# SCUT-BIP-Lab/SplatCo

Hardware: AMD Instinct MI355X
Metric: rasterizer fwd+bwd Msplats/s @1080p; PSNR-match vs ref (higher is better)
Workload: dtype f32; 1 GPU; cfg1: 1M synthetic Gaussians (seed 0), 1 view 1920x1080 per GPU, GaussianRasterizer forward+backward, colors_precomp + scale/rotation path; gaussians=1000000, image=1920x1080, visible=1000000, parallelism=1 view per GPU (mv sharding)

## Files before the change

include/splatco_raster.h:

```cpp
#ifndef SPLATCO_RASTER_H
#define SPLATCO_RASTER_H

#include <stddef.h>
#include <stdint.h>

#ifdef __cplusplus
extern "C" {
#endif

#define SCR_ABI_VERSION 36
#define SCR_TILE 16

typedef struct scr_settings {
    int32_t image_height;
    int32_t image_width;
    float tanfovx;
    float tanfovy;
    const float* bg;
    float scale_modifier;
    const float* viewmatrix;
    const float* projmatrix;
    int32_t sh_degree;
    const float* campos;
    int32_t prefiltered;
// ... 40 lines not shown
                 const void* binning_buf, void* image_buf, const float* dL_dcolor, const float* dL_ddepth,
                 const float* dL_dalpha, void* scratch,
                 float* dL_dmeans3D, float* dL_dmeans2D, float* dL_dcolors, float* dL_dsh,
                 float* dL_dopacity, float* dL_dscales, float* dL_drotations, float* dL_dcov3D,
                 float* dL_dviewmatrix, float* dL_dprojmatrix, float* dL_dcampos, void* stream);

enum {
    SCR_DBG_TILES_TOUCHED = 0,
    SCR_DBG_POINT_OFFSETS = 1,
    SCR_DBG_RANGES = 2,
    SCR_DBG_POINT_LIST = 3,
    SCR_DBG_N_CONTRIB = 4,
    SCR_DBG_FINAL_T = 5,
    SCR_DBG_SPLAT_RECORDS = 6,
    SCR_DBG_QMASK = 7,
    SCR_DBG_GM_INDEX = 8
};
int scr_debug_force_deep_lists(int mode);
int scr_debug_get(int which, int64_t P, int64_t num_rendered, int32_t image_height, int32_t image_width,
                  const void* geom_buf, const void* binning_buf, const void* image_buf, void* out,
                  void* stream);

size_t scr_tpa_scratch_bytes(int32_t R, int32_t H, int32_t W);
int scr_tpa_stats(int32_t R, int32_t H, int32_t W, const float* p0, const float* p1, const float* p2, float* avg,
                  float* mx, int32_t* arg, void* scratch, void* stream);
int scr_tpa_forward(int32_t R, int32_t H, int32_t W, const float* p0, const float* p1, const float* p2, const float* ca,
                    const float* w, float* s, uint8_t* am, float* sa, float* pair0, float* pair1, float* pair2, void* stream);
int scr_tpa_backward(int32_t R, int32_t H, int32_t W, const float* p0, const float* p1, const float* p2, const float* ca,
                     const float* w, const float* s, const uint8_t* am, const float* sa, const float* g0, const float* g1,
                     const float* g2, float* d0, float* d1, float* d2, float* dca, float* dw, void* scratch, void* stream);
int scr_tpa_backward_stats(int32_t R, int32_t H, int32_t W, const float* davg, const float* dmax, const int32_t* arg,
// ... 180 lines not shown
```

splatco_amd/_C.py:

```python
import ctypes as C
import os

import torch

_HERE = os.path.dirname(os.path.abspath(__file__))
LIB_PATH = os.environ.get("SPLATCO_RASTER_LIB", os.path.join(_HERE, "csrc", "libsplatco_raster.so"))

PLAN_NONFINITE_COLOUR, PLAN_LARGE_RECTS, PLAN_ANTIALIASED = 1, 2, 4
MODE_ANTIALIASED = 1
PROF_COUNT = 20
ABI_VERSION = 36
FLIP_MAX_RADIUS = 16

(DBG_TILES_TOUCHED, DBG_POINT_OFFSETS, DBG_RANGES, DBG_POINT_LIST, DBG_N_CONTRIB, DBG_FINAL_T, DBG_SPLAT_RECORDS, DBG_QMASK,
 DBG_GM_INDEX) = range(9)

vp, cp, u8, i32, i64, f32, f64, sz = C.c_void_p, C.c_char_p, C.c_uint8, C.c_int32, C.c_int64, C.c_float, C.c_double, C.c_size_t
P = C.POINTER


class Settings(C.Structure):
    _fields_ = [
        ("image_height", i32), ("image_width", i32),
        ("tanfovx", f32), ("tanfovy", f32),
        ("bg", vp), ("scale_modifier", f32),
        ("viewmatrix", vp), ("projmatrix", vp),
        ("sh_degree", i32), ("campos", vp),
        ("prefiltered", i32), ("debug", i32),
    ]

# ... 232 lines not shown
```

splatco_amd/csrc/binning.hip:

```cpp
#include "wg.h"

namespace scr {

__global__ void __launch_bounds__(1024) plan_scan_kernel(uint32_t nblk, uint32_t* __restrict__ block_sums,
                                                         unsigned long long* __restrict__ total,
                                                         uint32_t tiles, const uint32_t* __restrict__ tile_count,
                                                         uint32_t* __restrict__ ranges,
                                                         uint32_t* __restrict__ cursor,
                                                         volatile unsigned long long* mailbox,
                                                         unsigned long long seq) {
    __shared__ uint32_t lds[1024 / WAVE + 1];
    __shared__ unsigned long long wide[1024 / WAVE];
    if (blockIdx.x == 0) {
        unsigned long long carry = 0, mine = 0;
        for (uint32_t base = 0; base < nblk; base += 1024) {
            uint32_t i = base + threadIdx.x;
            uint32_t v = i < nblk ? block_sums[i] : 0u, tot;
            uint32_t ex = block_exclusive_scan<1024>(v, lds, tot);
            if (i < nblk) block_sums[i] = (uint32_t)carry + ex;
            carry += tot;
            mine += v;
        }
#pragma unroll
        for (int d = WAVE / 2; d > 0; d >>= 1) mine += (unsigned long long)__shfl_down((long long)mine, d, WAVE);
// ... 175 lines not shown
}
template <int E, int K>
__device__ __forceinline__ void bitonic_network(uint32_t (&klo)[E], uint32_t (&khi)[E], int lane) {
    bitonic_stage<E, K, K / 2>(klo, khi, lane);
    if constexpr (K < 64 * E) bitonic_network<E, K * 2>(klo, khi, lane);
}

constexpr int WAVE_SORT_MAX = 1024;

struct FinalLists {
    const uint2* gm_base;
    uint32_t* point_list;
    uint32_t* gm_index;
    uint8_t* qmask;
    int tx, ty;
    __device__ __forceinline__ void write(uint32_t i, uint32_t klo) const {
        const uint32_t id = klo >> 4;
        point_list[i] = id;
        qmask[i] = (uint8_t)(klo & 15u);
        if (gm_index) {
            const uint2 b = gm_base[id];
            gm_index[i] = b.x + (uint32_t)ty * b.y + (uint32_t)tx;
        }
    }
    template <int U, typename GetK>
    __device__ __forceinline__ void write_batch(uint32_t lo, uint32_t e0, uint32_t stride, uint32_t cnt, GetK getk) const {
        uint32_t k[U];
        uint2 b[U];
#pragma unroll
        for (int u = 0; u < U; ++u) {
            const uint32_t e = e0 + (uint32_t)u * stride;
            k[u] = e < cnt ? getk(e, u) : 0u;
        }
        if (gm_index) {
#pragma unroll
            for (int u = 0; u < U; ++u) b[u] = gm_base[k[u] >> 4];
        }
        __builtin_amdgcn_sched_barrier(0);
#pragma unroll
        for (int u = 0; u < U; ++u) {
            const uint32_t e = e0 + (uint32_t)u * stride;
            if (e < cnt) {
                point_list[lo + e] = k[u] >> 4;
                qmask[lo + e] = (uint8_t)(k[u] & 15u);
                if (gm_index) gm_index[lo + e] = b[u].x + (uint32_t)ty * b[u].y + (uint32_t)tx;
            }
        }
    }
};

template <int E>
__device__ __forceinline__ void wave_sort_regs(uint32_t n, const unsigned long long* __restrict__ keys,
                                               uint32_t (&klo)[E], uint32_t (&khi)[E]) {
    const int lane = threadIdx.x & 63;
#pragma unroll
    for (int e = 0; e < E; ++e) {
        const uint32_t i = (uint32_t)e * 64 + lane;
        const unsigned long long v = i < n ? keys[i] : ~0ull;
        klo[e] = (uint32_t)v;
        khi[e] = (uint32_t)(v >> 32);
    }
    bitonic_network<E, 2>(klo, khi, lane);
}

template <int E, bool FINAL>
__device__ __forceinline__ void wave_sort(uint32_t n, unsigned long long* __restrict__ keys, uint32_t lo,
                                          const FinalLists& fl, uint32_t* __restrict__ tr) {
    const int lane = threadIdx.x & 63;
    uint32_t klo[E], khi[E];
    wave_sort_regs<E>(n, keys, klo, khi);
    auto transpose = [&](uint32_t (&w)[E]) {
        __syncthreads();
#pragma unroll
        for (int e = 0; e < E; ++e) tr[lane * (E + 1) + e] = w[e];
        __syncthreads();
#pragma unroll
        for (int e = 0; e < E; ++e) {
            const int p = e * 64 + lane;
            w[e] = tr[p + p / E];
        }
    };
    transpose(klo);
    if (!FINAL) transpose(khi);
    if (FINAL) {
        fl.template write_batch<E>(lo, (uint32_t)lane, 64u, n, [&](uint32_t, int u) { return klo[u]; });
    } else {
#pragma unroll
        for (int e = 0; e < E; ++e) {
            const uint32_t i = (uint32_t)e * 64 + lane;
            if (i < n) keys[i] = ((unsigned long long)khi[e] << 32) | klo[e];
        }
    }
}

__device__ __forceinline__ int split_slot(int p) { return p + (p >> 3); }
constexpr int SPLIT_SLOTS = WAVE_SORT_MAX + WAVE_SORT_MAX / 8;
template <int EA, int EB>
__device__ __forceinline__ void wave_sort_split(uint32_t n, const unsigned long long* __restrict__ keys, uint32_t lo,
                                                const FinalLists& fl, unsigned long long* __restrict__ mb) {
    constexpr int NA = 64 * EA, NB = 64 * EB, PER = EA + EB;
    const int lane = threadIdx.x & 63;
    {
        uint32_t klo[EA], khi[EA];
        wave_sort_regs<EA>(NA, keys, klo, khi);
#pragma unroll
        for (int e = 0; e < EA; ++e) mb[split_slot(lane * EA + e)] = ((unsigned long long)khi[e] << 32) | klo[e];
    }
    {
        uint32_t klo[EB], khi[EB];
        wave_sort_regs<EB>(n - NA, keys + NA, klo, khi);
#pragma unroll
        for (int e = 0; e < EB; ++e) mb[split_slot(NA + lane * EB + e)] = ((unsigned long long)khi[e] << 32) | klo[e];
    }
// ... 17 lines not shown
            outk[k] = (uint32_t)(takeA ? x : y);
            if (takeA) {
                ++ia;
                x = ia < (uint32_t)NA ? keyA(ia) : ~0ull;
            } else {
                ++ib;
                y = ib < (uint32_t)NB ? keyB(ib) : ~0ull;
            }
        }
    }
    __syncthreads();
    uint32_t* tr = (uint32_t*)mb;
#pragma unroll
    for (int k = 0; k < PER; ++k) tr[lane * (PER + 1) + k] = outk[k];
    __syncthreads();
    fl.template write_batch<PER>(lo, (uint32_t)lane, 64u, n, [&](uint32_t i, int) { return tr[i + i / PER]; });
}

template <bool FINAL>
__device__ __forceinline__ void wave_sort_any(uint32_t n, unsigned long long* keys, uint32_t lo, const FinalLists& fl,
                                              unsigned long long* mb) {
    uint32_t* tr = (uint32_t*)mb;
    if (n <= 64) wave_sort<1, FINAL>(n, keys, lo, fl, tr);
    else if (n <= 128) wave_sort<2, FINAL>(n, keys, lo, fl, tr);
    else if (n <= 256) wave_sort<4, FINAL>(n, keys, lo, fl, tr);
    else if (FINAL && n > 256 && n <= 320) wave_sort_split<4, 1>(n, keys, lo, fl, mb);
    else if (FINAL && n > 256 && n <= 384) wave_sort_split<4, 2>(n, keys, lo, fl, mb);
    else if (n <= 512) wave_sort<8, FINAL>(n, keys, lo, fl, tr);
    else if (FINAL && n <= 576) wave_sort_split<8, 1>(n, keys, lo, fl, mb);
    else if (FINAL && n <= 640) wave_sort_split<8, 2>(n, keys, lo, fl, mb);
    else if (FINAL && n <= 768) wave_sort_split<8, 4>(n, keys, lo, fl, mb);
    else if (FINAL) wave_sort_split<8, 8>(n, keys, lo, fl, mb);
    else wave_sort<16, FINAL>(n, keys, lo, fl, tr);
}

__global__ void __launch_bounds__(64, 1)
tile_sort_wave_kernel(int tiles, int gx, const uint32_t* __restrict__ ranges, unsigned long long* __restrict__ keys,
                      const uint2* __restrict__ gm_base, uint32_t* __restrict__ point_list,
                      uint32_t* __restrict__ gm_index, uint8_t* __restrict__ qmask) {
    int t = xcd_tile(blockIdx.x, tiles);
    if (t < 0) return;
    const uint32_t lo = ranges[2 * t], n = ranges[2 * t + 1] - lo;
    if (n == 0 || n > (uint32_t)WAVE_SORT_MAX) return;
    const FinalLists fl{gm_base, point_list, gm_index, qmask, t % gx, t / gx};
    __shared__ unsigned long long mb[SPLIT_SLOTS];
    wave_sort_any<true>(n, keys + lo, lo, fl, mb);
}

constexpr int WG_SORT_THREADS = WG_SORT_MAX / 16;
__device__ __forceinline__ int wg_slot(int p) { return p + (p >> 4); }
__global__ void __launch_bounds__(WG_SORT_THREADS)
tile_sort_wg_kernel(int tiles, int gx, const uint32_t* __restrict__ ranges, unsigned long long* __restrict__ keys,
                    const uint2* __restrict__ gm_base, uint32_t* __restrict__ point_list,
                    uint32_t* __restrict__ gm_index, uint8_t* __restrict__ qmask) {
    extern __shared__ __attribute__((aligned(16))) unsigned long long buf[];
    int t = xcd_tile(blockIdx.x, tiles);
    if (t < 0) return;
    const uint32_t lo = ranges[2 * t], n = ranges[2 * t + 1] - lo;
    if (n <= (uint32_t)WAVE_SORT_MAX) return;
    const uint32_t c0 = blockIdx.y * (uint32_t)WG_SORT_MAX;
    if (c0 >= n) return;
// ... 184 lines not shown
            P, g.gx, g.tiles, gv.rec, gv.gm_base, gv.live_bits, gv.tiles_touched, gv.block_sums, gv.point_offsets, gv.ranges,
            gv.cursor, bv.keys, gv.total, cap_instances);
    else
        scatter_kernel<false><<<nb, BIN_THREADS, 0, st>>>(
            P, g.gx, g.tiles, gv.rec, gv.gm_base, gv.live_bits, gv.tiles_touched, gv.block_sums, gv.point_offsets, gv.ranges,
            gv.cursor, bv.keys, gv.total, cap_instances);
}

void launch_tile_sort(const KSettings& ks, const GeomView& gv, const BinView& bv, int64_t max_tile_instances,
                      bool with_gm_index, hipStream_t st) {
    uint32_t* const gm_index = with_gm_index ? bv.gm_index : nullptr;
    Grid g(ks.H, ks.W);
    const unsigned gt = (unsigned)xcd_grid(g.tiles);
    if (max_tile_instances <= 0) return;
    tile_sort_wave_kernel<<<gt, 64, 0, st>>>(g.tiles, g.gx, gv.ranges, bv.keys, gv.gm_base, bv.point_list, gm_index,
                                             bv.qmask);
    if (max_tile_instances <= WAVE_SORT_MAX) return;
    const unsigned chunks = (unsigned)((max_tile_instances + WG_SORT_MAX - 1) / WG_SORT_MAX);
    const size_t lds = (size_t)(WG_SORT_MAX + WG_SORT_MAX / 16) * 8;
    allow_dynamic_lds((const void*)tile_sort_wg_kernel, lds);
    tile_sort_wg_kernel<<<dim3(gt, chunks), WG_SORT_THREADS, lds, st>>>(g.tiles, g.gx, gv.ranges, bv.keys, gv.gm_base, bv.point_list,
                                                                        gm_index, bv.qmask);
    if (chunks <= 1) return;
    unsigned passes = 0;
    while ((1u << passes) < chunks) ++passes;
    const unsigned segs = (unsigned)((max_tile_instances + MP_SEG - 1) / MP_SEG);
    for (unsigned p = 0; p < passes; ++p) {
        const unsigned long long* src = (p & 1u) ? bv.keys2 : bv.keys;
        unsigned long long* dst = (p & 1u) ? bv.keys : bv.keys2;
        tile_merge_path_kernel<<<dim3(gt, segs), 256, 0, st>>>(g.tiles, g.gx, p, gv.ranges, src, dst, gv.gm_base,
                                                               bv.point_list, gm_index, bv.qmask);
// ... 5 lines not shown
```

splatco_amd/csrc/blend.hip:

```cpp
#include <type_traits>

#include "common.h"

namespace scr {

typedef float v2f __attribute__((ext_vector_type(2)));

#ifdef SCR_BLEND_COUNT
__device__ __forceinline__ void count_sub_blocks(unsigned long long m, unsigned long long (&len)[4]) {
    len[0] += (m & 0x000000000f0f0f0full) != 0ull;
    len[1] += (m & 0x00000000f0f0f0f0ull) != 0ull;
    len[2] += (m & 0x0f0f0f0f00000000ull) != 0ull;
    len[3] += (m & 0xf0f0f0f000000000ull) != 0ull;
}
#define SCR_COUNT_SUB(m) (count_sub_blocks((m), sub_), count_sub_blocks((m), subc_))
#define SCR_COUNT_CHUNK_END(i)                                                                             \
    do {                                                                                                   \
        const unsigned long long a_ = subc_[0] > subc_[1] ? subc_[0] : subc_[1], b_ = subc_[2] > subc_[3] ? subc_[2] : subc_[3]; \
        cnt_[(i)] += a_ > b_ ? a_ : b_;                                                                    \
        subc_[0] = subc_[1] = subc_[2] = subc_[3] = 0;                                                     \
    } while (0)
#define SCR_COUNT_SUB_FLUSH(i_sum, i_max)                                                                  \
    do {                                                                                                   \
        cnt_[(i_sum)] += sub_[0] + sub_[1] + sub_[2] + sub_[3];                                            \
// ... 389 lines not shown
}

template <bool AUX> struct RecTail { float x; };
template <> struct RecTail<true> { float x, z; };
constexpr int BCH = 64;
constexpr int BWD_MIN_WAVES = 4;
constexpr int ACC_BUFS = 2;

constexpr int BWD_MIN_WAVES_AUX = 3;
template <bool SAFE, bool AUX>
__global__ void __launch_bounds__(256, AUX ? BWD_MIN_WAVES_AUX : BWD_MIN_WAVES)
blend_backward_kernel(int W, int H, int gx, int tiles, const uint32_t* __restrict__ order, const unsigned long long* __restrict__ total,
                      const uint32_t* __restrict__ ranges,
                      const uint32_t* __restrict__ point_list, const uint32_t* __restrict__ gm_index,
                      const uint2* __restrict__ gm_base,
                      const uint8_t* __restrict__ qmask, const float4* __restrict__ rec,
                      const float* __restrict__ bg, const float* __restrict__ final_T,
                      const uint32_t* __restrict__ n_contrib, const float* __restrict__ dL_dpix,
                      GradRec* __restrict__ grad_rec, unsigned long long* __restrict__ cut_key, unsigned long long stamp,
                      uint8_t* __restrict__ has_rec, const float* __restrict__ dL_ddepth, const float* __restrict__ dL_dalpha,
                      float* __restrict__ grad_z) {
    __shared__ float4 st[4][3][BCH + 4];
    __shared__ float4 accA[ACC_BUFS][4][BCH], accB[ACC_BUFS][4][BCH];
    __shared__ float accC[ACC_BUFS][4][BCH];
    __shared__ float accD[ACC_BUFS][4][BCH];
    __shared__ __attribute__((aligned(16))) float tr[4][TR_WORDS];
    __shared__ uint32_t wave_max[4];
    const int t = blend_tile((int)blockIdx.x, tiles, order, total);
    if (t < 0) return;
    const uint32_t lo = ranges[2 * t], n = ranges[2 * t + 1] - lo;
    if (n == 0) return;
    const int wave = threadIdx.x >> 6, lane = threadIdx.x & 63;
    const int qx0 = (t % gx) * TILE + (wave & 1) * 8, qy0 = (t / gx) * TILE + (wave >> 1) * 8;
    const int px = qx0 + (lane >> 3), py = qy0 + (lane & 7);
    const bool inside = px < W && py < H;
    const float pxf = (float)px, pyf = (float)py;
    const float qx0f = (float)qx0, qy0f = (float)qy0;
    const size_t pix = (size_t)py * W + px, hw = (size_t)H * W;
    const uint32_t last = inside ? n_contrib[pix] : 0u;
    PixState ps;
    ps.T = inside ? final_T[pix] : 0.0f;
    ps.dLp0 = ps.dLp1 = ps.dLp2 = 0.0f;
    if (inside) {
        ps.dLp0 = dL_dpix[pix];
        ps.dLp1 = dL_dpix[hw + pix];
        ps.dLp2 = dL_dpix[2 * hw + pix];
// ... 37 lines not shown
    char* const rdst1 = rkind == 0 ? accA0 + 8 : rkind == 1 ? accA0 + 12 : accB0 + 12;
    char* const rdst2 = rkind == 0 ? accB0 + 4 : rkind == 1 ? accB0 : (char*)&accC[0][wave][0];
    const uint32_t rstride2 = rkind == 2 ? 4u : 16u;
    constexpr uint32_t PAR_A = sizeof(float4) * 4 * BCH, PAR_C = sizeof(float) * 4 * BCH;
    const uint32_t rpar2 = rkind == 2 ? PAR_C : PAR_A;
    uint32_t wm = last;
#pragma unroll
    for (int d = 32; d > 0; d >>= 1) wm = max(wm, (uint32_t)__shfl_xor((int)wm, d, WAVE));
    if (lane == 0) wave_max[wave] = wm;
    if (lane < 9) st[wave][lane / 3][lane % 3] = make_float4(0, 0, 0, 0);
    __syncthreads();
    const uint32_t wmax0 = wave_max[0], wmax1 = wave_max[1], wmax2 = wave_max[2], wmax3 = wave_max[3];
    const uint32_t max_last = max(max(wmax0, wmax1), max(wmax2, wmax3));
    const uint32_t wave_last = wave == 0 ? wmax0 : wave == 1 ? wmax1 : wave == 2 ? wmax2 : wmax3;
    const int nround = (int)((n + BCH - 1) / BCH);
    const int live_top = max_last ? (int)((max_last - 1) / BCH) : -1;

    constexpr int CUT_MIN_ROUNDS = 3;
    const bool cut = nround - 1 - live_top >= CUT_MIN_ROUNDS;
    if (threadIdx.x == 0) {
        unsigned long long ck = ~0ull;
        if (cut) {
            const uint32_t idc = point_list[lo + (uint32_t)(live_top + 1) * BCH];
            ck = ((unsigned long long)__float_as_uint(rec[3 * (size_t)idc + 2].y) << 32) | idc;
            cut_key[tiles] = stamp;
        }
        cut_key[t] = ck;
    }
    const uint32_t tile_x = (uint32_t)(t % gx), tile_y = (uint32_t)(t / gx);
    auto gm_of = [&](uint32_t pos, uint32_t id) -> uint32_t {
        if (gm_index) return gm_index[pos];
        const uint2 b = gm_base[id];
        return b.x + tile_y * b.y + tile_x;
    };
    if (!cut && (AUX || wave < 3))
        for (int ci = nround - 1; ci > live_top; --ci) {
            const uint32_t i = (uint32_t)ci * BCH + lane;
            if (i < n && qmask[lo + i] != 0) {
                const uint32_t gmi = gm_of(lo + i, point_list[lo + i]);
                GradRec& gr = grad_rec[gmi];
                if (wave == 0) store16_dword_aligned(&gr.a, make_float4(0, 0, 0, 0));
                else if (wave == 1) store16_dword_aligned(&gr.b, make_float4(0, 0, 0, 0));
                else if (!AUX || wave == 2) gr.c = 0.0f;
                else grad_z[gmi] = 0.0f;
            }
        }

    uint32_t m_next = 0, id_next = 0, slot_next = 0;
    uint32_t m_cur = 0, slot_cur = 0, id_cur = 0;
    bool sel_cur = false;
    float4 r0 = make_float4(0, 0, 0, 0), r1 = r0;
    RecTail<AUX> r2 = {};
    auto load_meta = [&](int ci, uint32_t& m, uint32_t& id, uint32_t& slot) {
        const uint32_t i = (uint32_t)ci * BCH + lane;
        const bool have = ci >= 0 && i < n;
        m = have ? qmask[lo + i] : 0u;
        id = have ? point_list[lo + i] : 0u;
        slot = have ? gm_of(lo + i, id) : 0u;
    };
    auto gather = [&](int ci, uint32_t m, uint32_t id, uint32_t slot) {
        const uint32_t i = (uint32_t)ci * BCH + lane;
        sel_cur = ((m >> wave) & 1u) && i < wave_last;
        m_cur = m;
        slot_cur = slot;
        id_cur = id;
        if (sel_cur) {
            r0 = rec[3 * (size_t)id];
            r1 = rec[3 * (size_t)id + 1];
            r2.x = rec[3 * (size_t)id + 2].x;
            if constexpr (AUX) r2.z = rec[3 * (size_t)id + 2].y;
        }
    };
    if (live_top >= 0) {
        uint32_t m0, id0, sl0;
        load_meta(live_top, m0, id0, sl0);
        gather(live_top, m0, id0, sl0);
        load_meta(live_top - 1, m_next, id_next, slot_next);
    }
    for (int ci = live_top; ci >= 0; --ci) {
        const uint32_t base = (uint32_t)ci * BCH;
        const int last_rel = (int)last - (int)base;
        const unsigned long long bal = __builtin_amdgcn_ballot_w64(sel_cur);
        const int cnt = __builtin_popcountll(bal);
        if (sel_cur) {
            const uint32_t pos = lanes_below(bal);
            st[wave][0][pos + 3] = r0;
            st[wave][1][pos + 3] = r1;
            float r2z = 0.0f;
            if constexpr (AUX) r2z = r2.z;
            st[wave][2][pos + 3] = make_float4(r2.x, __uint_as_float((uint32_t)lane), r2z, 0.0f);
        }
        const uint32_t m_this = m_cur, slot_this = slot_cur, id_this = id_cur;
        gather(ci - 1, m_next, id_next, slot_next);
        load_meta(ci - 2, m_next, id_next, slot_next);
        const int par = ci & 1;
        auto group = [&](const int k, auto tail) {
            constexpr bool TAIL = decltype(tail)::value;
            float Y[4], Wt[4];
            uint32_t jj[4] = {0u, 0u, 0u, 0u};
            unsigned long long hits[4] = {0ull, 0ull, 0ull, 0ull};
            float4 ra[4], rb[4];
            float2 rc[4];
            float rz[4] = {0.0f, 0.0f, 0.0f, 0.0f};
#pragma unroll
            for (int u = 0; u < 4; ++u) {
                ra[u] = st[wave][0][k + 3 - u];
                rb[u] = st[wave][1][k + 3 - u];
                rc[u] = *(const float2*)&st[wave][2][k + 3 - u];
                if (AUX) rz[u] = st[wave][2][k + 3 - u].z;
            }
            uint32_t jpos = 0u;
            if (BWD_LANE_POS) jpos = __float_as_uint(rpos[k].y);
            float Gs[4], al[4], om[4], Tu[4];
#pragma unroll
            for (int u = 0; u < 4; ++u) {
                if (TAIL && k - u < 0) {
                    Gs[u] = al[u] = 0.0f;
                    om[u] = 1.0f;
                    SCR_COUNT(13, 1);
                    continue;
                }
                const float4 a = ra[u], b = rb[u];
                const uint32_t j = __float_as_uint(rc[u].y);
                const float dx = a.x - pxf, dy = a.y - pyf;
                const float power = __builtin_fmaf(dx, __builtin_fmaf(a.z, dx, a.w * dy), (b.x * dy) * dy);
                const float ar = b.y * fast_exp(power);
                const unsigned long long hit = lanes((int)j < last_rel) & lanes(!(power > 0.0f)) & lanes(!(ar < 1.0f / 255.0f));
                SCR_COUNT(8, 1);
                SCR_COUNT(9, __builtin_popcountll(hit));
                SCR_COUNT_SUB(hit);
                SCR_COUNT(10, __builtin_popcountll(lanes(!((int)j < last_rel)) & lanes(inside)));
                SCR_COUNT(11, __builtin_popcountll(lanes(!(power > 0.0f)) & lanes(!(ar < 1.0f / 255.0f)) & lanes(inside)));
                Gs[u] = sel(hit, ar, 0.0f);
                al[u] = vmin(c099, Gs[u]);
                om[u] = 1.0f - al[u];
                if (SAFE) hits[u] = hit;
                jj[u] = j;
            }
            group_transmittance(ps.T, om, Tu);
#pragma unroll
            for (int u = 0; u < 4; ++u) {
                if (TAIL && k - u < 0) {
                    Y[u] = Wt[u] = 0.0f;
                    continue;
                }
                splat_pixel_grad<SAFE, AUX>(ps, Tu[u], rb[u], rc[u].x, rz[u], Gs[u], al[u], hits[u], Y[u], Wt[u]);
            }
            float s0, s1, s2;
            {
                asm volatile("" ::: "memory");
#pragma unroll
                for (int u = 0; u < 4; ++u) {
// ... 33 lines not shown
                const uint32_t jw = BWD_LANE_POS ? jpos : sel(rcu3, jj[3], sel(rcu2, jj[2], sel(rcu1, jj[1], jj[0])));
                *(float*)(rdst0 + par * PAR_A + jw * 16u) = s0;
                *(float*)(rdst1 + par * PAR_A + jw * 16u) = s1;
                *(float*)(rdst2 + par * rpar2 + jw * rstride2) = s2;
            }
            if (AUX && rstore_z && (!TAIL || k - rcu >= 0)) {
                const uint32_t jw = BWD_LANE_POS ? jpos : sel(rcu3, jj[3], sel(rcu2, jj[2], sel(rcu1, jj[1], jj[0])));
                accD[par][wave][jw] = s0;
            }
        };
        int k = cnt - 1;
        for (; k >= 3; k -= 4) group(k, std::false_type{});
        if (k >= 0) group(k, std::true_type{});
#ifdef SCR_BLEND_COUNT
        {
            const bool no_edge = ~(lanes(last_rel >= BCH) | lanes(last_rel <= 0)) == 0ull;
            SCR_COUNT(16, cnt != 0);
            SCR_COUNT(17, cnt != 0 && no_edge);
            SCR_COUNT(18, no_edge ? cnt : 0);
        }
#endif
        SCR_COUNT_CHUNK_END(7);
        asm volatile("s_waitcnt lgkmcnt(0)" ::: "memory");
        if (lane < cnt) {
            const float4 ra = st[wave][0][lane + 3];
            const uint32_t j = __float_as_uint(st[wave][2][lane + 3].y);
            const float a = ra.x - qx0f, b = ra.y - qy0f;
            const float4 A = accA[par][wave][j], B = accB[par][wave][j];
            const float M0 = A.x, Mx = A.y, My = A.z, Mxx = A.w, Mxy = B.x, Myy = B.y;
            const float t1 = a * M0 - Mx, t2 = b * M0 - My;
            accA[par][wave][j] = make_float4(t1, t2, a * (t1 - Mx) + Mxx, (a * t2 - b * Mx) + Mxy);
            accB[par][wave][j] = make_float4(b * (t2 - My) + Myy, M0, B.z, B.w);
        }
        __syncthreads();
        if (wave < 3 && base + lane < n && m_this != 0) {
            const uint32_t i = base + lane;
            float4 r = make_float4(0, 0, 0, 0);
            auto part = [&](int w) {
                return wave == 0 ? accA[par][w][lane] : wave == 1 ? accB[par][w][lane]
                                                                  : make_float4(accC[par][w][lane], 0.0f, 0.0f, 0.0f);
            };
            if constexpr (BWD_BATCH_COMBINE) {
                const unsigned long long took[4] = {lanes(((m_this >> 0) & 1u) && i < wmax0), lanes(((m_this >> 1) & 1u) && i < wmax1),
                                                    lanes(((m_this >> 2) & 1u) && i < wmax2), lanes(((m_this >> 3) & 1u) && i < wmax3)};
                if (wave == 2) {
                    const float x[4] = {accC[par][0][lane], accC[par][1][lane], accC[par][2][lane], accC[par][3][lane]};
                    masked_add4(r.x, x, took);
                } else {
                    const float4* const p = wave == 0 ? &accA[par][0][lane] : &accB[par][0][lane];
                    const float4 x[4] = {p[0], p[BCH], p[2 * BCH], p[3 * BCH]};
                    masked_add4(r, x, took);
                }
            } else {
            if (((m_this >> 0) & 1u) && i < wmax0) { const float4 x = part(0); r.x += x.x; r.y += x.y; r.z += x.z; r.w += x.w; }
            if (((m_this >> 1) & 1u) && i < wmax1) { const float4 x = part(1); r.x += x.x; r.y += x.y; r.z += x.z; r.w += x.w; }
            if (((m_this >> 2) & 1u) && i < wmax2) { const float4 x = part(2); r.x += x.x; r.y += x.y; r.z += x.z; r.w += x.w; }
            if (((m_this >> 3) & 1u) && i < wmax3) { const float4 x = part(3); r.x += x.x; r.y += x.y; r.z += x.z; r.w += x.w; }
            }
            GradRec& gr = grad_rec[slot_this];
            if (wave == 0) store16_dword_aligned(&gr.a, r);
            else if (wave == 1) store16_dword_aligned(&gr.b, r);
            else {
                gr.c = r.x;
                if (has_rec) has_rec[id_this] = 1;
            }
        }
        if (AUX && wave == 3 && base + lane < n && m_this != 0) {
            const uint32_t i = base + lane;
            float r = 0.0f;
            if constexpr (BWD_BATCH_COMBINE) {
                const unsigned long long took[4] = {lanes(((m_this >> 0) & 1u) && i < wmax0), lanes(((m_this >> 1) & 1u) && i < wmax1),
                                                    lanes(((m_this >> 2) & 1u) && i < wmax2), lanes(((m_this >> 3) & 1u) && i < wmax3)};
                const float x[4] = {accD[par][0][lane], accD[par][1][lane], accD[par][2][lane], accD[par][3][lane]};
                masked_add4(r, x, took);
            } else {
            if (((m_this >> 0) & 1u) && i < wmax0) r += accD[par][0][lane];
            if (((m_this >> 1) & 1u) && i < wmax1) r += accD[par][1][lane];
            if (((m_this >> 2) & 1u) && i < wmax2) r += accD[par][2][lane];
            if (((m_this >> 3) & 1u) && i < wmax3) r += accD[par][3][lane];
            }
            grad_z[slot_this] = r;
        }
    }
// ... 22 lines not shown
        ks.W, ks.H, g.gx, g.tiles, gv.tile_count, gv.total, gv.ranges, bv.point_list, bv.qmask, gv.rec, ks.bg, out_color, iv.final_T,
        iv.n_contrib, out_depth, out_alpha);
}

void launch_blend_backward(const KSettings& ks, const GeomView& gv, const BinView& bv, const ImgView& iv,
                           const float* dL_dcolor, const float* dL_ddepth, const float* dL_dalpha, GradRec* grad_rec,
                           float* grad_z, unsigned long long stamp, bool deep, bool flags, bool safe, hipStream_t st) {
    Grid g(ks.H, ks.W);
    const bool gm_from_base = deep;
    if (flags) { ZeroList z; z.add(gv.has_rec, ((size_t)gv.P + 3) / 4 * 4, st); launch_zero(z, st); }
    const bool aux = grad_z != nullptr;
    auto kernel = aux ? (safe ? blend_backward_kernel<true, true> : blend_backward_kernel<false, true>)
                      : (safe ? blend_backward_kernel<true, false> : blend_backward_kernel<false, false>);
    kernel<<<(unsigned)blend_slots_per_xcd(g) * NUM_XCD, 256, 0, st>>>(
        ks.W, ks.H, g.gx, g.tiles, gv.tile_count, gv.total, gv.ranges, bv.point_list, gm_from_base ? nullptr : bv.gm_index, gv.gm_base,
        bv.qmask, gv.rec, ks.bg,
        iv.final_T, iv.n_contrib, dL_dcolor, grad_rec, iv.cut_key, stamp, flags ? gv.has_rec : nullptr, dL_ddepth, dL_dalpha,
        grad_z);
}

}

#ifdef SCR_BLEND_COUNT
extern "C" int scr_tool_blend_counters(unsigned long long* out20, int reset) {
    if (out20 && hipMemcpyFromSymbol(out20, HIP_SYMBOL(scr::g_blend_counters), scr::SCR_NCOUNT * 8) != hipSuccess) return 1;
    if (reset) {
        unsigned long long z[scr::SCR_NCOUNT] = {};
        if (hipMemcpyToSymbol(HIP_SYMBOL(scr::g_blend_counters), z, scr::SCR_NCOUNT * 8) != hipSuccess) return 1;
    }
    return 0;
}
// ... 2 lines not shown
```

splatco_amd/csrc/capi.hip:

```cpp
#include <stdarg.h>
#include <stdio.h>
#include <string.h>

#include "capi.h"
#include <dlfcn.h>
#include <atomic>
#include <chrono>
#include <map>
#include <mutex>
#include <utility>
#include <vector>
#include <cstring>

using namespace scr;

static thread_local char g_err[512] = "";

namespace {
struct ProfRec { int idx; hipEvent_t a, b; };
unsigned g_prof_mask = 0;
unsigned g_prof_stride = 1;
unsigned g_prof_seen[32] = {};
std::vector<ProfRec> g_prof_recs;
std::vector<hipEvent_t> g_prof_pool;
// ... 366 lines not shown
}

int scr_debug_force_deep_lists(int mode) {
    if (mode < -1 || mode > 1) return fail("scr_debug_force_deep_lists: -1 (automatic), 0 or 1");
    scr::g_force_deep_lists = mode;
    return 0;
}

int scr_debug_get(int which, int64_t P, int64_t I, int32_t H, int32_t W, const void* geom_buf,
                  const void* binning_buf, const void* image_buf, void* out, void* stream) {
    SCR_MARK_FN;
    hipStream_t st = (hipStream_t)stream;
    Grid g(H, W);
    const void* src = nullptr;
    size_t bytes = 0;
    if (which <= SCR_DBG_RANGES || which == SCR_DBG_SPLAT_RECORDS) {
        if (!geom_buf) return fail("geom_buf is NULL");
        GeomView gv = geom_view((void*)geom_buf, P, H, W);
        if (which == SCR_DBG_TILES_TOUCHED) { src = gv.tiles_touched; bytes = (size_t)P * 4; }
        else if (which == SCR_DBG_POINT_OFFSETS) { src = gv.point_offsets; bytes = (size_t)P * 4; }
        else if (which == SCR_DBG_RANGES) { src = gv.ranges; bytes = (size_t)g.tiles * 8; }
        else { src = gv.rec; bytes = (size_t)P * REC_F * 4; }
    } else if (which == SCR_DBG_POINT_LIST) {
        if (!binning_buf) return fail("binning_buf is NULL");
        src = bin_view((void*)binning_buf, I, 0).point_list;
        bytes = (size_t)I * 4;
    } else if (which == SCR_DBG_QMASK || which == SCR_DBG_GM_INDEX) {
        if (!binning_buf) return fail("binning_buf is NULL");
        BinView bv = bin_view((void*)binning_buf, I, 0);
        if (which == SCR_DBG_GM_INDEX && deep_lists(I, g.tiles))
            return fail("gm_index is not materialised for deep tile lists (I > 8192 per tile on average)");
// ... 80 lines not shown
```

splatco_amd/csrc/common.h:

```cpp
#pragma once
#include <hip/hip_runtime.h>
#include <stdint.h>

#include "../../include/splatco_raster.h"

namespace scr {

__host__ __device__ __forceinline__ uint32_t sat_add_u32(uint32_t a, uint32_t b) {
    const uint32_t s = a + b;
    return s < a ? 0xFFFFFFFFu : s;
}


constexpr int TILE = SCR_TILE;
constexpr int TILE_PIX = TILE * TILE;
constexpr int WAVE = 64;
constexpr int NUM_XCD = 8;
constexpr int PRE_BLOCK = 256;
constexpr int BIN_THREADS = 1024;
constexpr int BIN_ROUNDS = 4;
constexpr int BIN_GPW = BIN_THREADS * BIN_ROUNDS;
constexpr int LDS_HIST_MAX_TILES = 40000;
constexpr int ID_BITS = 28;
constexpr int WG_SORT_MAX = 8192;
// ... 8 lines not shown
        : W(W_), H(H_), gx((W_ + TILE - 1) / TILE), gy((H_ + TILE - 1) / TILE), tiles(gx * gy) {}
};

struct GeomView {
    float4* rec;
    uint32_t* tiles_touched;
    uint32_t* point_offsets;
    uint8_t* clamped;
    uint2* gm_base;
    uint32_t* live_bits;
    uint8_t* has_rec;
    uint32_t* block_sums;
    uint32_t* tile_count;
    uint32_t* ranges;
    uint32_t* cursor;
    int64_t P;
    unsigned long long* total;
    size_t bytes;
};

inline __host__ GeomView geom_view(void* base, int64_t P, int H, int W) {
    Grid g(H, W);
    char* p = (char*)base;
    size_t off = 0;
    GeomView v;
    auto take = [&](size_t n) { char* q = p ? p + off : nullptr; off += align_up(n); return q; };
    size_t nblk = (size_t)((P + BIN_GPW - 1) / BIN_GPW);
    v.rec = (float4*)take((size_t)P * REC_F * 4);
    v.tiles_touched = (uint32_t*)take((size_t)P * 4);
    v.point_offsets = (uint32_t*)take((size_t)P * 4);
    v.clamped = (uint8_t*)take((size_t)P);
    v.gm_base = (uint2*)take((size_t)P * 8);
    v.live_bits = (uint32_t*)take((size_t)P * 4);
    v.has_rec = (uint8_t*)take((size_t)P);
    v.block_sums = (uint32_t*)take((nblk + 1) * 4);
    v.tile_count = (uint32_t*)take((size_t)g.tiles * 4);
    v.ranges = (uint32_t*)take((size_t)g.tiles * 8);
    v.cursor = (uint32_t*)take((size_t)g.tiles * 4);
    v.total = (unsigned long long*)take(128);
    v.bytes = off;
    v.P = P;
    return v;
}

extern int g_force_deep_lists;
inline __host__ bool deep_lists(int64_t I, int tiles) {
    return g_force_deep_lists >= 0 ? g_force_deep_lists != 0 : I > (int64_t)8192 * tiles;
}

constexpr int FLAGS_MIN_MEAN = 2048;
inline __host__ bool record_flags(int64_t I, int tiles) {
    return g_force_deep_lists >= 0 ? g_force_deep_lists != 0 : I > (int64_t)FLAGS_MIN_MEAN * tiles;
}

struct BinView {
    unsigned long long* keys;
    uint32_t* point_list;
    uint32_t* gm_index;
    uint8_t* qmask;
    unsigned long long* keys2;
    size_t bytes;
};

inline __host__ BinView bin_view(void* base, int64_t I, int64_t max_tile_instances) {
    char* p = (char*)base;
    size_t off = 0;
    BinView v;
    auto take = [&](size_t n) { char* q = p ? p + off : nullptr; off += align_up(n); return q; };
    size_t n = (size_t)(I > 0 ? I : 1);
    v.keys = (unsigned long long*)take(n * 8);
    v.point_list = (uint32_t*)take(n * 4);
    v.gm_index = (uint32_t*)take(n * 4);
    v.qmask = (uint8_t*)take(n);
    const bool merge = max_tile_instances > WG_SORT_MAX;
    v.keys2 = merge ? (unsigned long long*)take(n * 8) : nullptr;
    v.bytes = off;
    return v;
}

struct __attribute__((packed, aligned(4))) GradQuad { float x, y, z, w; };
struct __attribute__((packed, aligned(4))) GradRec { GradQuad a, b; float c; };
static_assert(sizeof(GradRec) == 36, "36-byte gradient records");
inline __host__ size_t grad_rec_bytes(int64_t I) { return align_up((size_t)(I > 0 ? I : 1) * sizeof(GradRec)); }
inline __host__ size_t grad_z_bytes(int64_t I) { return align_up((size_t)(I > 0 ? I : 1) * sizeof(float)); }

struct ImgView {
    float* final_T;
    uint32_t* n_contrib;
// ... 189 lines not shown
```

splatco_amd/rasterizer.py:

```python
from typing import NamedTuple

import ctypes as C
import os

import torch
import torch.nn as nn

from . import _C


class GaussianRasterizationSettings(NamedTuple):
    image_height: int
    image_width: int
    tanfovx: float
    tanfovy: float
    bg: torch.Tensor
    scale_modifier: float
    viewmatrix: torch.Tensor
    projmatrix: torch.Tensor
    sh_degree: int
    campos: torch.Tensor
    prefiltered: bool
    debug: bool

# ... 31 lines not shown


class RasterState:
    __slots__ = ("P", "M", "I", "max_tile", "flags", "cs", "geom", "binning", "image", "radii", "aux")

    def debug(self, which):
        dev = self.geom.device
        tiles = ((self.cs.W + 15) // 16) * ((self.cs.H + 15) // 16)
        shapes = {
            _C.DBG_TILES_TOUCHED: ((self.P,), torch.int32), _C.DBG_POINT_OFFSETS: ((self.P,), torch.int32),
            _C.DBG_RANGES: ((tiles, 2), torch.int32), _C.DBG_POINT_LIST: ((self.I,), torch.int32),
            _C.DBG_N_CONTRIB: ((self.cs.H, self.cs.W), torch.int32),
            _C.DBG_FINAL_T: ((self.cs.H, self.cs.W), torch.float32),
            _C.DBG_SPLAT_RECORDS: ((self.P, 12), torch.float32),
            _C.DBG_QMASK: ((self.I,), torch.uint8), _C.DBG_GM_INDEX: ((self.I,), torch.int32),
        }
        shape, dt = shapes[which]
        out = torch.empty(shape, dtype=dt, device=dev)
        if out.numel():
            _C.call("scr_debug_get", which, self.P, self.I, self.cs.H, self.cs.W, _C.ptr(self.geom), _C.ptr(self.binning),
                    _C.ptr(self.image), out)
        return out


SPECULATE = os.environ.get("SPLATCO_SPECULATIVE_BINNING", "1") != "0"
_plan_guess = {}


def rasterize_forward(cs, means3D, opacities, scales, rotations, cov3D_precomp, shs, colors_precomp, aux=False,
                      antialiased=False):
# ... 200 lines not shown
```

Before: 1120 Msplats/s.

## Compact live tile instances during final wave sort for backward blending

The final per-tile wave sort now also writes a compacted list of instances with a nonzero quadrant mask. Each entry is a pair of splat id and (original index << 4 | mask), written into the reused keys buffer, plus a per-tile live count. The backward blend kernel iterates only over these live entries and uses the stored original index for contribution-limit checks, so dead instances are no longer loaded and tested. This adds extra stores and a ballot during the sort and one more buffer of size I. Tiles that take the workgroup sort path fall back to the old uncompacted path.

```diff
diff --git a/include/splatco_raster.h b/include/splatco_raster.h
--- a/include/splatco_raster.h
+++ b/include/splatco_raster.h
@@ -78,7 +78,10 @@
     SCR_DBG_FINAL_T = 5,
     SCR_DBG_SPLAT_RECORDS = 6,
     SCR_DBG_QMASK = 7,
-    SCR_DBG_GM_INDEX = 8
+    SCR_DBG_GM_INDEX = 8,
+    SCR_DBG_LIVE_IDS = 9,
+    SCR_DBG_LIVE_WORDS = 10,
+    SCR_DBG_LIVE_COUNTS = 11
 };
 int scr_debug_force_deep_lists(int mode);
 int scr_debug_get(int which, int64_t P, int64_t num_rendered, int32_t image_height, int32_t image_width,
diff --git a/splatco_amd/_C.py b/splatco_amd/_C.py
--- a/splatco_amd/_C.py
+++ b/splatco_amd/_C.py
@@ -13,7 +13,7 @@
 FLIP_MAX_RADIUS = 16
 
 (DBG_TILES_TOUCHED, DBG_POINT_OFFSETS, DBG_RANGES, DBG_POINT_LIST, DBG_N_CONTRIB, DBG_FINAL_T, DBG_SPLAT_RECORDS, DBG_QMASK,
- DBG_GM_INDEX) = range(9)
+ DBG_GM_INDEX, DBG_LIVE_IDS, DBG_LIVE_WORDS, DBG_LIVE_COUNTS) = range(12)
 
 vp, cp, u8, i32, i64, f32, f64, sz = C.c_void_p, C.c_char_p, C.c_uint8, C.c_int32, C.c_int64, C.c_float, C.c_double, C.c_size_t
 P = C.POINTER
diff --git a/splatco_amd/csrc/binning.hip b/splatco_amd/csrc/binning.hip
--- a/splatco_amd/csrc/binning.hip
+++ b/splatco_amd/csrc/binning.hip
@@ -213,6 +213,8 @@
     uint32_t* gm_index;
     uint8_t* qmask;
     int tx, ty;
+    uint2* live_pair = nullptr;
+    uint32_t* live_gm = nullptr;
     __device__ __forceinline__ void write(uint32_t i, uint32_t klo) const {
         const uint32_t id = klo >> 4;
         point_list[i] = id;
@@ -222,8 +224,8 @@
             gm_index[i] = b.x + (uint32_t)ty * b.y + (uint32_t)tx;
         }
     }
-    template <int U, typename GetK>
-    __device__ __forceinline__ void write_batch(uint32_t lo, uint32_t e0, uint32_t stride, uint32_t cnt, GetK getk) const {
+    template <int U, bool LIVE = false, typename GetK>
+    __device__ __forceinline__ uint32_t write_batch(uint32_t lo, uint32_t e0, uint32_t stride, uint32_t cnt, GetK getk) const {
         uint32_t k[U];
         uint2 b[U];
 #pragma unroll
@@ -245,6 +247,24 @@
                 if (gm_index) gm_index[lo + e] = b[u].x + (uint32_t)ty * b[u].y + (uint32_t)tx;
             }
         }
+        uint32_t n_live = 0;
+        if constexpr (LIVE) {
+            {
+#pragma unroll
+                for (int u = 0; u < U; ++u) {
+                    const uint32_t e = e0 + (uint32_t)u * stride;
+                    const bool live = e < cnt && (k[u] & 15u) != 0u;
+                    const unsigned long long bal = __builtin_amdgcn_ballot_w64(live);
+                    if (live) {
+                        const uint32_t d = lo + n_live + lanes_below(bal);
+                        live_pair[d] = make_uint2(k[u] >> 4, (e << 4) | (k[u] & 15u));
+                        if (gm_index) live_gm[d] = b[u].x + (uint32_t)ty * b[u].y + (uint32_t)tx;
+                    }
+                    n_live += (uint32_t)__builtin_popcountll(bal);
+                }
+            }
+        }
+        return n_live;
     }
 };
 
@@ -263,7 +283,7 @@
 }
 
 template <int E, bool FINAL>
-__device__ __forceinline__ void wave_sort(uint32_t n, unsigned long long* __restrict__ keys, uint32_t lo,
+__device__ __forceinline__ uint32_t wave_sort(uint32_t n, unsigned long long* keys, uint32_t lo,
                                           const FinalLists& fl, uint32_t* __restrict__ tr) {
     const int lane = threadIdx.x & 63;
     uint32_t klo[E], khi[E];
@@ -282,7 +302,7 @@
     transpose(klo);
     if (!FINAL) transpose(khi);
     if (FINAL) {
-        fl.template write_batch<E>(lo, (uint32_t)lane, 64u, n, [&](uint32_t, int u) { return klo[u]; });
+        return fl.template write_batch<E, true>(lo, (uint32_t)lane, 64u, n, [&](uint32_t, int u) { return klo[u]; });
     } else {
 #pragma unroll
         for (int e = 0; e < E; ++e) {
@@ -290,12 +310,13 @@
             if (i < n) keys[i] = ((unsigned long long)khi[e] << 32) | klo[e];
         }
     }
+    return 0u;
 }
 
 __device__ __forceinline__ int split_slot(int p) { return p + (p >> 3); }
 constexpr int SPLIT_SLOTS = WAVE_SORT_MAX + WAVE_SORT_MAX / 8;
 template <int EA, int EB>
-__device__ __forceinline__ void wave_sort_split(uint32_t n, const unsigned long long* __restrict__ keys, uint32_t lo,
+__device__ __forceinline__ uint32_t wave_sort_split(uint32_t n, const unsigned long long* keys, uint32_t lo,
                                                 const FinalLists& fl, unsigned long long* __restrict__ mb) {
     constexpr int NA = 64 * EA, NB = 64 * EB, PER = EA + EB;
     const int lane = threadIdx.x & 63;
@@ -343,37 +364,42 @@
 #pragma unroll
     for (int k = 0; k < PER; ++k) tr[lane * (PER + 1) + k] = outk[k];
     __syncthreads();
-    fl.template write_batch<PER>(lo, (uint32_t)lane, 64u, n, [&](uint32_t i, int) { return tr[i + i / PER]; });
+    return fl.template write_batch<PER, true>(lo, (uint32_t)lane, 64u, n, [&](uint32_t i, int) { return tr[i + i / PER]; });
 }
 
 template <bool FINAL>
-__device__ __forceinline__ void wave_sort_any(uint32_t n, unsigned long long* keys, uint32_t lo, const FinalLists& fl,
+__device__ __forceinline__ uint32_t wave_sort_any(uint32_t n, unsigned long long* keys, uint32_t lo, const FinalLists& fl,
                                               unsigned long long* mb) {
     uint32_t* tr = (uint32_t*)mb;
-    if (n <= 64) wave_sort<1, FINAL>(n, keys, lo, fl, tr);
-    else if (n <= 128) wave_sort<2, FINAL>(n, keys, lo, fl, tr);
-    else if (n <= 256) wave_sort<4, FINAL>(n, keys, lo, fl, tr);
-    else if (FINAL && n > 256 && n <= 320) wave_sort_split<4, 1>(n, keys, lo, fl, mb);
-    else if (FINAL && n > 256 && n <= 384) wave_sort_split<4, 2>(n, keys, lo, fl, mb);
-    else if (n <= 512) wave_sort<8, FINAL>(n, keys, lo, fl, tr);
-    else if (FINAL && n <= 576) wave_sort_split<8, 1>(n, keys, lo, fl, mb);
-    else if (FINAL && n <= 640) wave_sort_split<8, 2>(n, keys, lo, fl, mb);
-    else if (FINAL && n <= 768) wave_sort_split<8, 4>(n, keys, lo, fl, mb);
-    else if (FINAL) wave_sort_split<8, 8>(n, keys, lo, fl, mb);
-    else wave_sort<16, FINAL>(n, keys, lo, fl, tr);
+    if (n <= 64) return wave_sort<1, FINAL>(n, keys, lo, fl, tr);
+    if (n <= 128) return wave_sort<2, FINAL>(n, keys, lo, fl, tr);
+    if (n <= 256) return wave_sort<4, FINAL>(n, keys, lo, fl, tr);
+    if (FINAL && n > 256 && n <= 320) return wave_sort_split<4, 1>(n, keys, lo, fl, mb);
+    if (FINAL && n > 256 && n <= 384) return wave_sort_split<4, 2>(n, keys, lo, fl, mb);
+    if (n <= 512) return wave_sort<8, FINAL>(n, keys, lo, fl, tr);
+    if (FINAL && n <= 576) return wave_sort_split<8, 1>(n, keys, lo, fl, mb);
+    if (FINAL && n <= 640) return wave_sort_split<8, 2>(n, keys, lo, fl, mb);
+    if (FINAL && n <= 768) return wave_sort_split<8, 4>(n, keys, lo, fl, mb);
+    if (FINAL) return wave_sort_split<8, 8>(n, keys, lo, fl, mb);
+    return wave_sort<16, FINAL>(n, keys, lo, fl, tr);
 }
 
 __global__ void __launch_bounds__(64, 1)
-tile_sort_wave_kernel(int tiles, int gx, const uint32_t* __restrict__ ranges, unsigned long long* __restrict__ keys,
+tile_sort_wave_kernel(int tiles, int gx, const uint32_t* __restrict__ ranges, unsigned long long* keys,
                       const uint2* __restrict__ gm_base, uint32_t* __restrict__ point_list,
-                      uint32_t* __restrict__ gm_index, uint8_t* __restrict__ qmask) {
+                      uint32_t* __restrict__ gm_index, uint8_t* __restrict__ qmask,
+                      uint32_t* __restrict__ live_gm, uint32_t* __restrict__ live_count) {
     int t = xcd_tile(blockIdx.x, tiles);
     if (t < 0) return;
     const uint32_t lo = ranges[2 * t], n = ranges[2 * t + 1] - lo;
-    if (n == 0 || n > (uint32_t)WAVE_SORT_MAX) return;
-    const FinalLists fl{gm_base, point_list, gm_index, qmask, t % gx, t / gx};
+    if (n == 0 || n > (uint32_t)WAVE_SORT_MAX) {
+        if (threadIdx.x == 0) live_count[t] = n == 0 ? 0u : LIVE_NONE;
+        return;
+    }
+    const FinalLists fl{gm_base, point_list, gm_index, qmask, t % gx, t / gx, (uint2*)keys, live_gm};
     __shared__ unsigned long long mb[SPLIT_SLOTS];
-    wave_sort_any<true>(n, keys + lo, lo, fl, mb);
+    const uint32_t n_live = wave_sort_any<true>(n, keys + lo, lo, fl, mb);
+    if (threadIdx.x == 0) live_count[t] = n_live;
 }
 
 constexpr int WG_SORT_THREADS = WG_SORT_MAX / 16;
@@ -588,7 +614,7 @@
     const unsigned gt = (unsigned)xcd_grid(g.tiles);
     if (max_tile_instances <= 0) return;
     tile_sort_wave_kernel<<<gt, 64, 0, st>>>(g.tiles, g.gx, gv.ranges, bv.keys, gv.gm_base, bv.point_list, gm_index,
-                                             bv.qmask);
+                                             bv.qmask, bv.live_gm, gv.live_count);
     if (max_tile_instances <= WAVE_SORT_MAX) return;
     const unsigned chunks = (unsigned)((max_tile_instances + WG_SORT_MAX - 1) / WG_SORT_MAX);
     const size_t lds = (size_t)(WG_SORT_MAX + WG_SORT_MAX / 16) * 8;
diff --git a/splatco_amd/csrc/blend.hip b/splatco_amd/csrc/blend.hip
--- a/splatco_amd/csrc/blend.hip
+++ b/splatco_amd/csrc/blend.hip
@@ -427,7 +427,9 @@
                       const uint32_t* __restrict__ ranges,
                       const uint32_t* __restrict__ point_list, const uint32_t* __restrict__ gm_index,
                       const uint2* __restrict__ gm_base,
-                      const uint8_t* __restrict__ qmask, const float4* __restrict__ rec,
+                      const uint8_t* __restrict__ qmask, const uint32_t* __restrict__ live_count,
+                      const uint2* __restrict__ live_pair, const uint32_t* __restrict__ live_gm,
+                      const float4* __restrict__ rec,
                       const float* __restrict__ bg, const float* __restrict__ final_T,
                       const uint32_t* __restrict__ n_contrib, const float* __restrict__ dL_dpix,
                       GradRec* __restrict__ grad_rec, unsigned long long* __restrict__ cut_key, unsigned long long stamp,
@@ -441,8 +443,15 @@
     __shared__ uint32_t wave_max[4];
     const int t = blend_tile((int)blockIdx.x, tiles, order, total);
     if (t < 0) return;
-    const uint32_t lo = ranges[2 * t], n = ranges[2 * t + 1] - lo;
-    if (n == 0) return;
+    const uint32_t lo = ranges[2 * t], n_raw = ranges[2 * t + 1] - lo;
+    if (n_raw == 0) return;
+    const uint32_t nlv = live_count[t];
+    const bool compact = nlv != LIVE_NONE;
+    const uint32_t n = compact ? nlv : n_raw;
+    if (n == 0) {
+        if (threadIdx.x == 0) cut_key[t] = ~0ull;
+        return;
+    }
     const int wave = threadIdx.x >> 6, lane = threadIdx.x & 63;
     const int qx0 = (t % gx) * TILE + (wave & 1) * 8, qy0 = (t / gx) * TILE + (wave >> 1) * 8;
     const int px = qx0 + (lane >> 3), py = qy0 + (lane & 7);
@@ -510,14 +519,18 @@
     const uint32_t max_last = max(max(wmax0, wmax1), max(wmax2, wmax3));
     const uint32_t wave_last = wave == 0 ? wmax0 : wave == 1 ? wmax1 : wave == 2 ? wmax2 : wmax3;
     const int nround = (int)((n + BCH - 1) / BCH);
-    const int live_top = max_last ? (int)((max_last - 1) / BCH) : -1;
+    int live_top = max_last ? (int)((max_last - 1) / BCH) : -1;
+    if (compact) {
+        const bool first_in = lane < nround && (live_pair[lo + (uint32_t)lane * BCH].y >> 4) < max_last;
+        live_top = __builtin_popcountll(__builtin_amdgcn_ballot_w64(first_in)) - 1;
+    }
 
     constexpr int CUT_MIN_ROUNDS = 3;
     const bool cut = nround - 1 - live_top >= CUT_MIN_ROUNDS;
     if (threadIdx.x == 0) {
         unsigned long long ck = ~0ull;
         if (cut) {
-            const uint32_t idc = point_list[lo + (uint32_t)(live_top + 1) * BCH];
+            const uint32_t idc = compact ? live_pair[lo + (uint32_t)(live_top + 1) * BCH].x : point_list[lo + (uint32_t)(live_top + 1) * BCH];
             ck = ((unsigned long long)__float_as_uint(rec[3 * (size_t)idc + 2].y) << 32) | idc;
             cut_key[tiles] = stamp;
         }
@@ -532,8 +545,8 @@
     if (!cut && (AUX || wave < 3))
         for (int ci = nround - 1; ci > live_top; --ci) {
             const uint32_t i = (uint32_t)ci * BCH + lane;
-            if (i < n && qmask[lo + i] != 0) {
-                const uint32_t gmi = gm_of(lo + i, point_list[lo + i]);
+            if (i < n && (compact || qmask[lo + i] != 0)) {
+                const uint32_t gmi = compact && gm_index ? live_gm[lo + i] : gm_of(lo + i, (compact ? live_pair[lo + i].x : point_list[lo + i]));
                 GradRec& gr = grad_rec[gmi];
                 if (wave == 0) store16_dword_aligned(&gr.a, make_float4(0, 0, 0, 0));
                 else if (wave == 1) store16_dword_aligned(&gr.b, make_float4(0, 0, 0, 0));
@@ -550,13 +563,19 @@
     auto load_meta = [&](int ci, uint32_t& m, uint32_t& id, uint32_t& slot) {
         const uint32_t i = (uint32_t)ci * BCH + lane;
         const bool have = ci >= 0 && i < n;
-        m = have ? qmask[lo + i] : 0u;
-        id = have ? point_list[lo + i] : 0u;
-        slot = have ? gm_of(lo + i, id) : 0u;
+        if (compact) {
+            const uint2 p = have ? live_pair[lo + i] : make_uint2(0u, 0u);
+            id = p.x;
+            m = p.y;
+            slot = have ? (gm_index ? live_gm[lo + i] : gm_of(0u, id)) : 0u;
+        } else {
+            m = have ? (i << 4) | qmask[lo + i] : 0u;
+            id = have ? point_list[lo + i] : 0u;
+            slot = have ? gm_of(lo + i, id) : 0u;
+        }
     };
-    auto gather = [&](int ci, uint32_t m, uint32_t id, uint32_t slot) {
-        const uint32_t i = (uint32_t)ci * BCH + lane;
-        sel_cur = ((m >> wave) & 1u) && i < wave_last;
+    auto gather = [&](uint32_t m, uint32_t id, uint32_t slot) {
+        sel_cur = ((m >> wave) & 1u) && (m >> 4) < wave_last;
         m_cur = m;
         slot_cur = slot;
         id_cur = id;
@@ -570,12 +589,11 @@
     if (live_top >= 0) {
         uint32_t m0, id0, sl0;
         load_meta(live_top, m0, id0, sl0);
-        gather(live_top, m0, id0, sl0);
+        gather(m0, id0, sl0);
         load_meta(live_top - 1, m_next, id_next, slot_next);
     }
     for (int ci = live_top; ci >= 0; --ci) {
         const uint32_t base = (uint32_t)ci * BCH;
-        const int last_rel = (int)last - (int)base;
         const unsigned long long bal = __builtin_amdgcn_ballot_w64(sel_cur);
         const int cnt = __builtin_popcountll(bal);
         if (sel_cur) {
@@ -584,10 +602,10 @@
             st[wave][1][pos + 3] = r1;
             float r2z = 0.0f;
             if constexpr (AUX) r2z = r2.z;
-            st[wave][2][pos + 3] = make_float4(r2.x, __uint_as_float((uint32_t)lane), r2z, 0.0f);
+            st[wave][2][pos + 3] = make_float4(r2.x, __uint_as_float(m_cur >> 4), r2z, __uint_as_float((uint32_t)lane));
         }
         const uint32_t m_this = m_cur, slot_this = slot_cur, id_this = id_cur;
-        gather(ci - 1, m_next, id_next, slot_next);
+        gather(m_next, id_next, slot_next);
         load_meta(ci - 2, m_next, id_next, slot_next);
         const int par = ci & 1;
         auto group = [&](const int k, auto tail) {
@@ -606,7 +624,7 @@
                 if (AUX) rz[u] = st[wave][2][k + 3 - u].z;
             }
             uint32_t jpos = 0u;
-            if (BWD_LANE_POS) jpos = __float_as_uint(rpos[k].y);
+            if (BWD_LANE_POS) jpos = __float_as_uint(rpos[k].w);
             float Gs[4], al[4], om[4], Tu[4];
 #pragma unroll
             for (int u = 0; u < 4; ++u) {
@@ -621,17 +639,17 @@
                 const float dx = a.x - pxf, dy = a.y - pyf;
                 const float power = __builtin_fmaf(dx, __builtin_fmaf(a.z, dx, a.w * dy), (b.x * dy) * dy);
                 const float ar = b.y * fast_exp(power);
-                const unsigned long long hit = lanes((int)j < last_rel) & lanes(!(power > 0.0f)) & lanes(!(ar < 1.0f / 255.0f));
+                const unsigned long long hit = lanes(j < last) & lanes(!(power > 0.0f)) & lanes(!(ar < 1.0f / 255.0f));
                 SCR_COUNT(8, 1);
                 SCR_COUNT(9, __builtin_popcountll(hit));
                 SCR_COUNT_SUB(hit);
-                SCR_COUNT(10, __builtin_popcountll(lanes(!((int)j < last_rel)) & lanes(inside)));
+                SCR_COUNT(10, __builtin_popcountll(lanes(!(j < last)) & lanes(inside)));
                 SCR_COUNT(11, __builtin_popcountll(lanes(!(power > 0.0f)) & lanes(!(ar < 1.0f / 255.0f)) & lanes(inside)));
                 Gs[u] = sel(hit, ar, 0.0f);
                 al[u] = vmin(c099, Gs[u]);
                 om[u] = 1.0f - al[u];
                 if (SAFE) hits[u] = hit;
-                jj[u] = j;
+                if (!BWD_LANE_POS) jj[u] = __float_as_uint(st[wave][2][k + 3 - u].w);
             }
             group_transmittance(ps.T, om, Tu);
 #pragma unroll
@@ -695,7 +713,10 @@
         if (k >= 0) group(k, std::true_type{});
 #ifdef SCR_BLEND_COUNT
         {
-            const bool no_edge = ~(lanes(last_rel >= BCH) | lanes(last_rel <= 0)) == 0ull;
+            const uint32_t cntw = min((uint32_t)BCH, n - base);
+            const uint32_t p_first = (uint32_t)__builtin_amdgcn_readfirstlane((int)(m_this >> 4));
+            const uint32_t p_last = (uint32_t)__builtin_amdgcn_readlane((int)(m_this >> 4), (int)cntw - 1);
+            const bool no_edge = ~(lanes(last > p_last) | lanes(last <= p_first)) == 0ull;
             SCR_COUNT(16, cnt != 0);
             SCR_COUNT(17, cnt != 0 && no_edge);
             SCR_COUNT(18, no_edge ? cnt : 0);
@@ -705,7 +726,7 @@
         asm volatile("s_waitcnt lgkmcnt(0)" ::: "memory");
         if (lane < cnt) {
             const float4 ra = st[wave][0][lane + 3];
-            const uint32_t j = __float_as_uint(st[wave][2][lane + 3].y);
+            const uint32_t j = __float_as_uint(st[wave][2][lane + 3].w);
             const float a = ra.x - qx0f, b = ra.y - qy0f;
             const float4 A = accA[par][wave][j], B = accB[par][wave][j];
             const float M0 = A.x, Mx = A.y, My = A.z, Mxx = A.w, Mxy = B.x, Myy = B.y;
@@ -714,8 +735,8 @@
             accB[par][wave][j] = make_float4(b * (t2 - My) + Myy, M0, B.z, B.w);
         }
         __syncthreads();
-        if (wave < 3 && base + lane < n && m_this != 0) {
-            const uint32_t i = base + lane;
+        if (wave < 3 && base + lane < n && (m_this & 15u) != 0) {
+            const uint32_t i = m_this >> 4;
             float4 r = make_float4(0, 0, 0, 0);
             auto part = [&](int w) {
                 return wave == 0 ? accA[par][w][lane] : wave == 1 ? accB[par][w][lane]
@@ -746,8 +767,8 @@
                 if (has_rec) has_rec[id_this] = 1;
             }
         }
-        if (AUX && wave == 3 && base + lane < n && m_this != 0) {
-            const uint32_t i = base + lane;
+        if (AUX && wave == 3 && base + lane < n && (m_this & 15u) != 0) {
+            const uint32_t i = m_this >> 4;
             float r = 0.0f;
             if constexpr (BWD_BATCH_COMBINE) {
                 const unsigned long long took[4] = {lanes(((m_this >> 0) & 1u) && i < wmax0), lanes(((m_this >> 1) & 1u) && i < wmax1),
@@ -800,7 +821,7 @@
                       : (safe ? blend_backward_kernel<true, false> : blend_backward_kernel<false, false>);
     kernel<<<(unsigned)blend_slots_per_xcd(g) * NUM_XCD, 256, 0, st>>>(
         ks.W, ks.H, g.gx, g.tiles, gv.tile_count, gv.total, gv.ranges, bv.point_list, gm_from_base ? nullptr : bv.gm_index, gv.gm_base,
-        bv.qmask, gv.rec, ks.bg,
+        bv.qmask, gv.live_count, bv.live_pair, bv.live_gm, gv.rec, ks.bg,
         iv.final_T, iv.n_contrib, dL_dcolor, grad_rec, iv.cut_key, stamp, flags ? gv.has_rec : nullptr, dL_ddepth, dL_dalpha,
         grad_z);
 }
diff --git a/splatco_amd/csrc/capi.hip b/splatco_amd/csrc/capi.hip
--- a/splatco_amd/csrc/capi.hip
+++ b/splatco_amd/csrc/capi.hip
@@ -404,7 +404,15 @@
     Grid g(H, W);
     const void* src = nullptr;
     size_t bytes = 0;
-    if (which <= SCR_DBG_RANGES || which == SCR_DBG_SPLAT_RECORDS) {
+    if (which == SCR_DBG_LIVE_COUNTS) {
+        if (!geom_buf) return fail("geom_buf is NULL");
+        src = geom_view((void*)geom_buf, P, H, W).live_count;
+        bytes = (size_t)g.tiles * 4;
+    } else if (which == SCR_DBG_LIVE_IDS || which == SCR_DBG_LIVE_WORDS) {
+        if (!binning_buf) return fail("binning_buf is NULL");
+        if (I > 0) HIP_TRY(hipMemcpy2DAsync(out, 4, (const uint32_t*)bin_view((void*)binning_buf, I, 0).live_pair + (which == SCR_DBG_LIVE_WORDS), 8, 4,
+                                            (size_t)I, hipMemcpyDeviceToDevice, st));
+    } else if (which <= SCR_DBG_RANGES || which == SCR_DBG_SPLAT_RECORDS) {
         if (!geom_buf) return fail("geom_buf is NULL");
         GeomView gv = geom_view((void*)geom_buf, P, H, W);
         if (which == SCR_DBG_TILES_TOUCHED) { src = gv.tiles_touched; bytes = (size_t)P * 4; }
diff --git a/splatco_amd/csrc/common.h b/splatco_amd/csrc/common.h
--- a/splatco_amd/csrc/common.h
+++ b/splatco_amd/csrc/common.h
@@ -46,6 +46,7 @@
     uint32_t* tile_count;
     uint32_t* ranges;
     uint32_t* cursor;
+    uint32_t* live_count;
     int64_t P;
     unsigned long long* total;
     size_t bytes;
@@ -69,6 +70,7 @@
     v.tile_count = (uint32_t*)take((size_t)g.tiles * 4);
     v.ranges = (uint32_t*)take((size_t)g.tiles * 8);
     v.cursor = (uint32_t*)take((size_t)g.tiles * 4);
+    v.live_count = (uint32_t*)take((size_t)g.tiles * 4);
     v.total = (unsigned long long*)take(128);
     v.bytes = off;
     v.P = P;
@@ -90,9 +92,12 @@
     uint32_t* point_list;
     uint32_t* gm_index;
     uint8_t* qmask;
+    uint2* live_pair;
+    uint32_t* live_gm;
     unsigned long long* keys2;
     size_t bytes;
 };
+constexpr uint32_t LIVE_NONE = 0xFFFFFFFFu;
 
 inline __host__ BinView bin_view(void* base, int64_t I, int64_t max_tile_instances) {
     char* p = (char*)base;
@@ -104,6 +109,8 @@
     v.point_list = (uint32_t*)take(n * 4);
     v.gm_index = (uint32_t*)take(n * 4);
     v.qmask = (uint8_t*)take(n);
+    v.live_pair = (uint2*)v.keys;
+    v.live_gm = (uint32_t*)take(n * 4);
     const bool merge = max_tile_instances > WG_SORT_MAX;
     v.keys2 = merge ? (unsigned long long*)take(n * 8) : nullptr;
     v.bytes = off;
diff --git a/splatco_amd/rasterizer.py b/splatco_amd/rasterizer.py
--- a/splatco_amd/rasterizer.py
+++ b/splatco_amd/rasterizer.py
@@ -69,6 +69,8 @@
             _C.DBG_FINAL_T: ((self.cs.H, self.cs.W), torch.float32),
             _C.DBG_SPLAT_RECORDS: ((self.P, 12), torch.float32),
             _C.DBG_QMASK: ((self.I,), torch.uint8), _C.DBG_GM_INDEX: ((self.I,), torch.int32),
+            _C.DBG_LIVE_IDS: ((self.I,), torch.int32), _C.DBG_LIVE_WORDS: ((self.I,), torch.int32),
+            _C.DBG_LIVE_COUNTS: ((tiles,), torch.int32),
         }
         shape, dt = shapes[which]
         out = torch.empty(shape, dtype=dt, device=dev)
```

Result: no change. 1129 Msplats/s, median of 6 (+0.8%).
